# Jax-Rene/monitor-systam-flink-quickstart

Hardware: AMD Instinct MI355X
Metric: events/sec (node) + p50 alert latency, 1M-key tumbling window at 1/2/4/8 MI355X (higher is better)
Workload: dtype int64; 1 GPU; global_batch=16777216, seq_len=60000, parallelism=keyBy-a2a1, exchange=none, keyed_state=dense, record_bytes=8, keys=1000000, key_distribution=uniform, device=cuda:0

## Files before the change

csrc/kernels_hip.hip:

```cpp
#include <hip/hip_runtime.h>

#include <cstdlib>

#include <algorithm>
#include <numeric>
#include <stdexcept>
#include <string>

#include "mxs_hip_util.h"
#include "mxs_kernels.h"

namespace mxs {
namespace {

constexpr int kWave = 64;

__device__ __forceinline__ int lane_id() { return threadIdx.x & (kWave - 1); }

__device__ __forceinline__ int64_t wave_max_i64(int64_t v) {
#pragma unroll
  for (int o = 32; o > 0; o >>= 1) {
    int64_t w = __shfl_xor(v, o);
    v = v > w ? v : w;
  }
// ... 770 lines not shown
    if (simple) {
      bool ok = true;
#pragma unroll
      for (int u = 0; u < CU; ++u) {
        const int64_t d = ct[u] - plan.tbase;
        ok = ok && ck[u] < kTombKey && !(plan.drop_late && ct[u] < plan.late_ts) && d >= 0 &&
             d < ((int64_t)1 << 31);
      }
      simple = __all(ok);
    }
    if (RB == 8 && simple) {
#pragma unroll
      for (int u = 0; u < CU; ++u) {
        const uint64_t k = ck[u];
        const int64_t t = ct[u];
        const uint64_t v = cv[u];
        tmax = t > tmax ? t : tmax;
        const uint32_t du = (uint32_t)(t - plan.tbase);
        uint32_t q = (uint32_t)((double)du * plan.inv_pane);
        const uint32_t qp = q * pane_u;
        q = qp > du ? q - 1u : (du - qp >= pane_u ? q + 1u : q);
        qmin32 = q < qmin32 ? q : qmin32;
        pmask |= pane_bit(q);
        qmax32 = q > qmax32 ? q : qmax32;
        flags |= (int64_t)(int32_t)v != (int64_t)v ? 4 : 0;
        uint32_t b;
        if constexpr (ONE) {
          b = sub_of(k, plan);
        } else {
          const int32_t jh = plan.nranks == 1 ? 0
                             : plan.hash_mode ? jhash_tab[k] : java_long_hash((int64_t)k);
          b = kg_lds ? bucket_of(k, jh, plan, skg) : bucket_of(k, jh, plan, kg_dest);
        }
        keep[u] = true;
        bk[u] = b;
        if constexpr (RB == 8) {
          flags |= narrow_fits(k, (int64_t)v, q) ? 0 : 16;
          rec[u] = make_uint2((uint32_t)k, ((uint32_t)v << 4) | (q & 15u));
        } else {
          rec[u] = make_uint4((uint32_t)k, (uint32_t)(k >> 32), (uint32_t)v, q);
        }
        rk[u] = atomicAdd(&rcnt[b], 1u);
      }
    } else
#pragma unroll
    for (int u = 0; u < CU; ++u) {
      const int64_t i = ev_at(r0, u);
      keep[u] = false;
      if (i < end) {
        const uint64_t k = ck[u];
        const int64_t t = ct[u];
        const uint64_t v = cv[u];
        tmax = t > tmax ? t : tmax;
        const PartEval e = ONE      ? part_eval<true>(k, t, jhash_tab, plan, kg_dest)
                           : kg_lds ? part_eval(k, t, jhash_tab, plan, skg)
                                    : part_eval(k, t, jhash_tab, plan, kg_dest);
        if (e.kind == 1) {
          ++nlate;
          if (late_idx) {
            const unsigned long long pos = atomicAdd((unsigned long long*)&stats[kStatLate], 1ull);
            if (pos < late_cap) late_idx[pos] = (uint32_t)i;
          }
        } else if (e.kind >= 2) {
          flags |= e.kind == 2 ? 2 : 8;
        } else {
          if ((int64_t)(int32_t)v != (int64_t)v) flags |= 4;
          qmin32 = e.t < qmin32 ? e.t : qmin32;
          pmask |= pane_bit(e.t);
          qmax32 = e.t > qmax32 ? e.t : qmax32;
          keep[u] = true;
          bk[u] = e.bucket;
          if constexpr (RB == 8) {
            if (!narrow_fits(k, (int64_t)v, e.t)) flags |= 16;
            rec[u] = make_uint2((uint32_t)k, ((uint32_t)v << 4) | (e.t & 15u));
          } else {
            rec[u] = make_uint4((uint32_t)k, (uint32_t)(k >> 32), (uint32_t)v, e.t);
          }
          rk[u] = atomicAdd(&rcnt[e.bucket], 1u);
        }
      }
    }
    __syncthreads();
    const uint32_t myc = threadIdx.x < (unsigned)nb ? rcnt[threadIdx.x] : 0u;
    const uint32_t off = block_exclusive_scan(myc, wsum);
    if (threadIdx.x < (unsigned)nb) {
      roff[threadIdx.x] = off;
      dbase[threadIdx.x] = threadIdx.x * bcap + run_base[threadIdx.x] + lcnt[threadIdx.x] - off;
    }
    __syncthreads();
#pragma unroll
    for (int u = 0; u < CU; ++u)
      if (keep[u]) {
        const uint32_t j = roff[bk[u]] + rk[u];
        rbuf[j] = rec[u];
        sbk[j] = (uint16_t)bk[u];
      }
    __syncthreads();
    const uint32_t nrec = wsum[16];
    nacc += threadIdx.x == 0 ? nrec : 0u;
    if (!any_ovf) {
      RT* outr = (RT*)out;
      for (uint32_t j = threadIdx.x; j < nrec; j += blockDim.x) outr[dbase[sbk[j]] + j] = rbuf[j];
    }
    __syncthreads();
    if (threadIdx.x < (unsigned)nb) {
      lcnt[threadIdx.x] += rcnt[threadIdx.x];
      rcnt[threadIdx.x] = 0;
    }
    __syncthreads();
  }
  if (threadIdx.x < (unsigned)nb && !any_ovf) {
    const int b = threadIdx.x;
    RT* dst = (RT*)out + (size_t)b * bcap + run_base[b];
    RT hole;
    if constexpr (RB == 8) hole = make_uint2(0xFFFFFFFFu, 0xFFFFFFFFu);
    else hole = make_uint4(0xFFFFFFFFu, 0xFFFFFFFFu, 0u, kHoleT);
    for (uint32_t w = lcnt[b]; w < resv[b]; ++w) dst[w] = hole;
  }

  int64_t qmin = qmin32 == 0xFFFFFFFFu && qmax32 == 0 ? INT64_MAX : (int64_t)qmin32;
  int64_t qmax = qmin == INT64_MAX ? INT64_MIN : (int64_t)qmax32;
  tmax = block_reduce_i64(tmax, lred, 0);
  qmin = block_reduce_i64(qmin, lred, 1);
  qmax = block_reduce_i64(qmax, lred, 0);
  pmask = (uint32_t)block_reduce_i64(pmask, lred, 3);
  if (!late_idx) nlate = block_reduce_i64(nlate, lred, 2);
  flags = (any_ovf ? 1 : 0) | block_reduce_i64(flags & 2, lred, 0) |
          block_reduce_i64(flags & 4, lred, 0) | block_reduce_i64(flags & 8, lred, 0) |
          (RB == 8 ? block_reduce_i64(flags & 16, lred, 0) : 0);
  if (threadIdx.x == 0) {
    atomicMax((long long*)&stats[kStatMaxTs], (long long)tmax);
    if (nacc) {
      atomicMin((long long*)&stats[kStatMinPane], (long long)qmin);
      atomicMax((long long*)&stats[kStatMaxPane], (long long)qmax);
      atomicAdd((unsigned long long*)&stats[kStatAccepted], (unsigned long long)nacc);
      if (pmask) atomicOr((unsigned long long*)&stats[kStatPaneMask], (unsigned long long)pmask);
    }
    if (!late_idx && nlate) atomicAdd((unsigned long long*)&stats[kStatLate], (unsigned long long)nlate);
    if (flags) atomicOr((unsigned long long*)&stats[kStatOverflow], (unsigned long long)flags);
  }
}

constexpr int kOpSub = 4;
__device__ __forceinline__ uint32_t wave_inclusive_scan_dpp(uint32_t x) {
  x += (uint32_t)__builtin_amdgcn_update_dpp(0, (int)x, 0x111, 0xF, 0xF, false);
  x += (uint32_t)__builtin_amdgcn_update_dpp(0, (int)x, 0x112, 0xF, 0xF, false);
  x += (uint32_t)__builtin_amdgcn_update_dpp(0, (int)x, 0x114, 0xF, 0xF, false);
  x += (uint32_t)__builtin_amdgcn_update_dpp(0, (int)x, 0x118, 0xF, 0xF, false);
  x += (uint32_t)__builtin_amdgcn_update_dpp(0, (int)x, 0x142, 0xA, 0xF, false);
  x += (uint32_t)__builtin_amdgcn_update_dpp(0, (int)x, 0x143, 0xC, 0xF, false);
  return x;
}
constexpr size_t onepass_lds(int ru) {
  return (size_t)1024 * ru * 8 + (size_t)(3 * kCMaxNb + 4) * 4 + 20 * 4 + 16 * 8;
}
static_assert(kCG == kPartGranule, "reservation granule differs from the host's capacity bound");
static_assert(onepass_lds(kOnePassRound / 1024) <= 160 * 1024, "one-pass round exceeds 160 KiB");

template <int V, int RU, bool K32, bool PAIR>
__global__ __launch_bounds__(1024) void partition_onepass_kernel(
    const uint64_t* __restrict__ keys, const int64_t* __restrict__ ts,
    const uint64_t* __restrict__ vals, int64_t n, int64_t chunk, PartPlan plan,
    uint32_t* __restrict__ cursor, uint2* __restrict__ out, int64_t* __restrict__ stats,
    uint32_t* __restrict__ late_idx, uint32_t late_cap) {
  static_assert(RU % kOpSub == 0, "a round is a whole number of sub-steps");
  constexpr int R = 1024 * RU, NS = RU / kOpSub, SUB = 1024 * kOpSub;
  constexpr uint32_t kDropped = 0xFFFFFFFFu;
  extern __shared__ __attribute__((aligned(16))) unsigned char osm[];
  const int nb = 1 << plan.nsub_log2;
  uint2* rbuf = (uint2*)osm;
  uint32_t* rcnt = (uint32_t*)(rbuf + R);
  uint32_t* roff = rcnt + kCMaxNb;
  uint32_t* gbase = roff + kCMaxNb + 4;
  uint32_t* wsum = gbase + kCMaxNb;
  int64_t* lred = (int64_t*)(wsum + 20);

  for (int b = threadIdx.x; b < kCMaxNb; b += blockDim.x) rcnt[b] = 0;
  if (threadIdx.x == 0) {
    wsum[17] = 0;
    wsum[18] = 0;
    wsum[19] = 0;
  }
  __syncthreads();
  const int64_t start = (int64_t)blockIdx.x * chunk;
  const int64_t end = start + chunk < n ? start + chunk : n;
  const uint32_t bcap = plan.bucket_cap;

  auto tid_now = [&]() -> uint32_t {
    uint32_t t = threadIdx.x;
    asm volatile("" : "+v"(t));
    return t;
  };
  auto ev_off = [&](int u) -> uint32_t {
    if constexpr (PAIR) return (uint32_t)(u >> 1) * 2048u + 2u * tid_now() + (uint32_t)(u & 1);
    else return (uint32_t)u * 1024u + tid_now();
  };
  auto sub_len = [&](int64_t base) -> uint32_t {
    const int64_t rem = end - base;
    return rem <= 0 ? 0u : rem >= SUB ? (uint32_t)SUB : (uint32_t)rem;
  };
  uint64_t nk[kOpSub], nv[kOpSub];
  int64_t nt[kOpSub];
  auto load_half = [&](int64_t base, int h) {
    const uint32_t len = sub_len(base);
    const uint64_t* kb = K32 ? reinterpret_cast<const uint64_t*>(
                                   reinterpret_cast<const int32_t*>(keys) + base)
                             : keys + base;
    const int64_t* tb = ts + base;
    const uint64_t* vb = vals + base;
    if constexpr (PAIR) {
      {
        const int u = 2 * h;
        const uint32_t o = ev_off(u);
        if (o + 1 < len) {
          ldkey2<V, K32>(kb, o, nk[u], nk[u + 1]);
          uint64_t t0, t1;
          ld64x2<V>(tb, o, t0, t1);
          nt[u] = (int64_t)t0;
          nt[u + 1] = (int64_t)t1;
          ld64x2<V>(vb, o, nv[u], nv[u + 1]);
        } else if (o < len) {
          nk[u] = ldkey<V, K32>(kb, o);
          nt[u] = ldin<V>(&tb[o]);
          nv[u] = ldin<V>(&vb[o]);
        }
      }
    } else {
#pragma unroll
      for (int u = 2 * h; u < 2 * h + 2; ++u) {
        const uint32_t o = ev_off(u);
        if (o < len) {
          nk[u] = ldkey<V, K32>(kb, o);
          nt[u] = ldin<V>(&tb[o]);
          nv[u] = ldin<V>(&vb[o]);
        }
      }
    }
  };
  static_assert(kOpSub == 4, "a sub-step is two halves of two events");

  int64_t tmax = INT64_MIN;
  uint32_t nlate = 0, qmin32 = 0xFFFFFFFFu, qmax32 = 0, pmask = 0, flags = 0;
  const bool pane32 = plan.window_mode && plan.pane > 0 && plan.pane < ((int64_t)1 << 31);
  const uint32_t pane_u = (uint32_t)plan.pane;
  load_half(start, 0);
  load_half(start, 1);
  for (int64_t r0 = start; r0 < end; r0 += R) {
    uint2 rec[RU];
    uint32_t br[RU];
#pragma unroll
    for (int s = 0; s < NS; ++s) {
      const int64_t s0 = r0 + (int64_t)s * SUB;
      const uint32_t len = sub_len(s0);
      bool simple = len == (uint32_t)SUB && pane32 && !(plan.ablate & 8u);
      if (simple) {
        int64_t tbase_v = plan.tbase;
        asm volatile("" : "+s"(tbase_v));
        bool ok = true;
#pragma unroll
        for (int u = 0; u < kOpSub; ++u) {
          const int64_t d = nt[u] - tbase_v;
          ok = ok && nk[u] < kTombKey && !(plan.drop_late && nt[u] < plan.late_ts) && d >= 0 &&
               d < ((int64_t)1 << 31);
        }
        simple = __all(ok);
      }
      if (simple) {
#pragma unroll
        for (int u = 0; u < kOpSub; ++u) {
          const uint64_t k = nk[u];
          const int64_t t = nt[u];
          const uint64_t v = nv[u];
          tmax = t > tmax ? t : tmax;
          const uint32_t du = (uint32_t)(t - plan.tbase);
          uint32_t q = (uint32_t)((double)du * plan.inv_pane);
          const uint32_t qp = q * pane_u;
          q = qp > du ? q - 1u : (du - qp >= pane_u ? q + 1u : q);
          qmin32 = q < qmin32 ? q : qmin32;
          pmask |= pane_bit(q);
          qmax32 = q > qmax32 ? q : qmax32;
          flags |= (int64_t)(int32_t)v != (int64_t)v ? 4u : 0u;
          flags |= narrow_fits(k, (int64_t)v, q) ? 0u : 16u;
          const uint32_t b = sub_of(k, plan);
          rec[s * kOpSub + u] = make_uint2((uint32_t)k, ((uint32_t)v << 4) | (q & 15u));
          br[s * kOpSub + u] = (b << 16) | atomicAdd(&rcnt[b], 1u);
          if (u & 1) load_half(s0 + SUB, u >> 1);
          __builtin_amdgcn_sched_barrier(0);
        }
      } else {
#pragma unroll 1
        for (int u = 0; u < kOpSub; ++u) {
          uint64_t k = nk[0], v = nv[0];
          int64_t t = nt[0];
#pragma unroll
          for (int j = 1; j < kOpSub; ++j)
            if (u == j) {
              k = nk[j];
              t = nt[j];
              v = nv[j];
            }
          uint32_t rx = 0, ry = 0, rb = kDropped;
          const uint32_t o = ev_off(u);
          if (o < len) {
            tmax = t > tmax ? t : tmax;
            const PartEval e = part_eval<true>(k, t, nullptr, plan, nullptr);
            if (e.kind == 1) {
              ++nlate;
              if (late_idx) {
                const unsigned long long pos =
                    atomicAdd((unsigned long long*)&stats[kStatLate], 1ull);
                if (pos < late_cap) late_idx[pos] = (uint32_t)(s0 + o);
              }
            } else if (e.kind >= 2) {
              flags |= e.kind == 2 ? 2u : 8u;
            } else {
              if ((int64_t)(int32_t)v != (int64_t)v) flags |= 4u;
              qmin32 = e.t < qmin32 ? e.t : qmin32;
              pmask |= pane_bit(e.t);
              qmax32 = e.t > qmax32 ? e.t : qmax32;
              if (!narrow_fits(k, (int64_t)v, e.t)) flags |= 16u;
              rx = (uint32_t)k;
              ry = ((uint32_t)v << 4) | (e.t & 15u);
              rb = (e.bucket << 16) | atomicAdd(&rcnt[e.bucket], 1u);
            }
          }
#pragma unroll
          for (int j = 0; j < kOpSub; ++j)
            if (u == j) {
              rec[s * kOpSub + j] = make_uint2(rx, ry);
              br[s * kOpSub + j] = rb;
            }
        }
        load_half(s0 + SUB, 0);
        load_half(s0 + SUB, 1);
      }
    }
    __syncthreads();
    const uint32_t tid = tid_now();
    if (tid < 64) {
      const uint4 c0 = ((const uint4*)rcnt)[2 * tid];
      const uint4 c1 = ((const uint4*)rcnt)[2 * tid + 1];
      ((uint4*)rcnt)[2 * tid] = make_uint4(0, 0, 0, 0);
      ((uint4*)rcnt)[2 * tid + 1] = make_uint4(0, 0, 0, 0);
      const uint32_t sum = c0.x + c0.y + c0.z + c0.w + c1.x + c1.y + c1.z + c1.w;
      const uint32_t incl = wave_inclusive_scan_dpp(sum);
      uint4 o0, o1;
      o0.x = incl - sum;
      o0.y = o0.x + c0.x;
      o0.z = o0.y + c0.y;
      o0.w = o0.z + c0.z;
      o1.x = o0.w + c0.w;
      o1.y = o1.x + c1.x;
      o1.z = o1.y + c1.y;
      o1.w = o1.z + c1.z;
      ((uint4*)roff)[2 * tid] = o0;
      ((uint4*)roff)[2 * tid + 1] = o1;
      if (tid == 63) {
        roff[kCMaxNb] = incl;
        wsum[17] += incl;
      }
    }
    __syncthreads();
    uint32_t c4 = 0, gb = 0;
    if (tid < (unsigned)nb) {
      c4 = (roff[tid + 1] - roff[tid] + (kCG - 1)) & ~(uint32_t)(kCG - 1);
      if (c4) gb = atomicAdd(&cursor[tid], c4);
    }
#pragma unroll
    for (int u = 0; u < RU; ++u)
      if (br[u] != kDropped) rbuf[roff[br[u] >> 16] + (br[u] & 0xFFFFu)] = rec[u];
    if (tid < (unsigned)nb) {
      if (c4) {
        if ((uint64_t)gb + c4 > bcap) wsum[18] = 1;
        atomicMax(&wsum[19], gb + c4);
      }
      gbase[tid] = tid * bcap + gb;
    }
    __syncthreads();
    if (!wsum[18]) {
      const int lane = lane_id();
      for (int b = tid >> 6; b < nb; b += 16) {
        const uint32_t o = roff[b], cnt = roff[b + 1] - o;
        const uint32_t cr = (cnt + (kCG - 1)) & ~(uint32_t)(kCG - 1);
        uint4* dst = (uint4*)(out + gbase[b]);
        for (uint32_t j = 2 * lane; j < cr; j += 128) {
          const uint2 a = j < cnt ? rbuf[o + j] : make_uint2(0xFFFFFFFFu, 0xFFFFFFFFu);
          const uint2 c = j + 1 < cnt ? rbuf[o + j + 1] : make_uint2(0xFFFFFFFFu, 0xFFFFFFFFu);
          dst[j >> 1] = make_uint4(a.x, a.y, c.x, c.y);
        }
      }
    }
  }
  __syncthreads();
  const bool any_ovf = wsum[18] != 0;
  const uint32_t nacc = wsum[17];

  int64_t qmin = qmin32 == 0xFFFFFFFFu && qmax32 == 0 ? INT64_MAX : (int64_t)qmin32;
  int64_t qmax = qmin == INT64_MAX ? INT64_MIN : (int64_t)qmax32;
  tmax = block_reduce_i64(tmax, lred, 0);
  qmin = block_reduce_i64(qmin, lred, 1);
  qmax = block_reduce_i64(qmax, lred, 0);
  pmask = (uint32_t)block_reduce_i64(pmask, lred, 3);
  const int64_t nlate_g = late_idx ? 0 : block_reduce_i64(nlate, lred, 2);
  const int64_t fl = (any_ovf ? 1 : 0) | block_reduce_i64(flags, lred, 3);
  if (threadIdx.x == 0) {
    if (wsum[19])
      atomicMax((unsigned long long*)&stats[kStatMaxBucket], (unsigned long long)wsum[19]);
    atomicMax((long long*)&stats[kStatMaxTs], (long long)tmax);
    if (nacc) {
      atomicMin((long long*)&stats[kStatMinPane], (long long)qmin);
      atomicMax((long long*)&stats[kStatMaxPane], (long long)qmax);
      atomicAdd((unsigned long long*)&stats[kStatAccepted], (unsigned long long)nacc);
      if (pmask) atomicOr((unsigned long long*)&stats[kStatPaneMask], (unsigned long long)pmask);
    }
    if (nlate_g) atomicAdd((unsigned long long*)&stats[kStatLate], (unsigned long long)nlate_g);
    if (fl) atomicOr((unsigned long long*)&stats[kStatOverflow], (unsigned long long)fl);
  }
}

__global__ __launch_bounds__(256) void step_begin_kernel(uint32_t* __restrict__ cursor, int nb,
                                                         int64_t* __restrict__ stats) {
  for (int i = blockIdx.x * blockDim.x + threadIdx.x; i < nb; i += gridDim.x * blockDim.x)
    cursor[i] = 0;
  if (blockIdx.x == 0 && threadIdx.x < kStatCount) {
    const int j = threadIdx.x;
    stats[j] = j == kStatMaxTs ? INT64_MIN : j == kStatMinPane ? INT64_MAX
             : j == kStatMaxPane ? INT64_MIN : 0;
  }
}

__global__ void step_finish_kernel(const int64_t* __restrict__ stats, int64_t* __restrict__ local_maxts,
                                   int64_t bound, int32_t event_mode, int64_t proc_now,
                                   int64_t* __restrict__ red, const uint32_t* __restrict__ flags,
                                   int32_t idle, int64_t* __restrict__ host_red, int32_t fill_word,
                                   const uint32_t* __restrict__ cursor, int nb,
                                   uint32_t* __restrict__ next_cursor,
                                   int64_t* __restrict__ next_stats) {
  if (next_cursor) {
    for (int i = threadIdx.x; i < nb; i += blockDim.x) next_cursor[i] = 0;
    if (threadIdx.x < kStatCount) {
      const int j = threadIdx.x;
      next_stats[j] = j == kStatMaxTs ? INT64_MIN : j == kStatMinPane ? INT64_MAX
                    : j == kStatMaxPane ? INT64_MIN : 0;
    }
  }
  __shared__ uint32_t fmax[64];
  if (fill_word) {
    uint32_t m = 0;
    for (int i = threadIdx.x; i < nb; i += 64) m = cursor[i] > m ? cursor[i] : m;
    fmax[threadIdx.x] = m;
    __syncthreads();
    for (int s = 32; s > 0; s >>= 1) {
      if ((int)threadIdx.x < s && fmax[threadIdx.x + s] > fmax[threadIdx.x])
        fmax[threadIdx.x] = fmax[threadIdx.x + s];
      __syncthreads();
    }
  }
  const int j = threadIdx.x;
  if (j >= 16) return;
  int64_t lm = local_maxts[0];
  const int64_t bm = stats[kStatMaxTs];
  lm = bm > lm ? bm : lm;
  if (j == 0) local_maxts[0] = lm;
  const int64_t wm = event_mode ? (lm == INT64_MIN ? INT64_MIN : lm - bound) : proc_now;
  const int64_t ovf = stats[kStatOverflow];
  int64_t v;
  switch (j) {
    case 0: {
      const int64_t qmax = stats[kStatMaxPane];
      v = qmax == INT64_MIN ? INT64_MAX : -qmax;
      break;
    }
    case 1: v = stats[kStatMinPane]; break;
    case 2: v = idle ? INT64_MAX : wm; break;
    case 3:
      v = !fill_word ? -(ovf & 1) : (ovf & 1) ? -((int64_t)1 << 40) : -(int64_t)fmax[0];
      break;
    case 4: v = -((ovf >> 1) & 1); break;
    case 5: v = (ovf & 4) ? -2 : (ovf & 16) ? -1 : 0; break;
    case 6: v = flags ? -(int64_t)(flags[0] & 1u) : 0; break;
    case 7: v = -((ovf >> 3) & 1); break;
    default: v = stats[j - 8]; break;
  }
  red[j] = v;
  if (host_red) host_red[j] = v;
}

__global__ __launch_bounds__(256) void combine_check_kernel(const uint32_t* __restrict__ flags,
                                                            const uint32_t* __restrict__ counts,
                                                            int nb, int64_t* __restrict__ chk) {
  __shared__ uint32_t mx[256];
  __shared__ uint64_t sm[256];
  uint32_t m = 0;
  uint64_t sum = 0;
  for (int i = threadIdx.x; i < nb; i += 256) {
    m = counts[i] > m ? counts[i] : m;
    sum += counts[i];
  }
  mx[threadIdx.x] = m;
  sm[threadIdx.x] = sum;
  __syncthreads();
  for (int s = 128; s > 0; s >>= 1) {
    if ((int)threadIdx.x < s) {
      if (mx[threadIdx.x + s] > mx[threadIdx.x]) mx[threadIdx.x] = mx[threadIdx.x + s];
      sm[threadIdx.x] += sm[threadIdx.x + s];
    }
    __syncthreads();
  }
  if (threadIdx.x == 0) {
    chk[0] = -(int64_t)(flags[0] & 2u);
    chk[1] = -(int64_t)mx[0];
    chk[2] = (int64_t)sm[0];
  }
}

__global__ __launch_bounds__(256) void bucket_repack_kernel(const uint64_t* __restrict__ src,
                                                            const uint32_t* __restrict__ counts,
                                                            uint32_t src_cap, uint32_t dst_cap,
                                                            int words, uint64_t* __restrict__ dst,
                                                            unsigned long long* __restrict__ xstat) {
  const int b = blockIdx.x;
  const uint32_t c = counts[b] < dst_cap ? counts[b] : dst_cap;
  const uint64_t* s = src + (size_t)b * src_cap * words;
  uint64_t* d = dst + (size_t)b * dst_cap * words;
  const size_t nw = (size_t)c * words;
  if (!(((uintptr_t)s | (uintptr_t)d) & 15)) {
    const size_t nv = nw / 2;
    const uint4* s4 = (const uint4*)s;
    uint4* d4 = (uint4*)d;
    for (size_t i = threadIdx.x; i < nv; i += blockDim.x) d4[i] = s4[i];
    if ((nw & 1) && threadIdx.x == 0) d[nw - 1] = s[nw - 1];
  } else {
    for (size_t i = threadIdx.x; i < nw; i += blockDim.x) d[i] = s[i];
  }
  if (xstat && threadIdx.x == 0) {
    atomicAdd(&xstat[1], (unsigned long long)nw * 8ull);
    atomicAdd(&xstat[0], (unsigned long long)dst_cap * words * 8ull);
  }
}

__global__ __launch_bounds__(256) void neg_max_u32_kernel(const uint32_t* __restrict__ counts, int nb,
                                                          int64_t* __restrict__ out) {
  __shared__ uint32_t mx[256];
  uint32_t m = 0;
  for (int i = threadIdx.x; i < nb; i += 256) m = counts[i] > m ? counts[i] : m;
  mx[threadIdx.x] = m;
  __syncthreads();
  for (int s = 128; s > 0; s >>= 1) {
// ... 3420 lines not shown
    }
  }
  auto kfn = partition_compact_kernel<1, kCUProd, ONE, RB, K32, PAIR>;
  static bool attr = false;
  if (!attr) {
    MXS_HIP_CHECK(hipFuncSetAttribute((const void*)kfn, hipFuncAttributeMaxDynamicSharedMemorySize,
                                      (int)compact_lds(kCUProd)));
    attr = true;
  }
  const size_t lds = compact_lds(kCUProd) - (ONE ? (size_t)kKgLdsMax * 4 : 0);
  hipLaunchKernelGGL(kfn, dim3(blocks), dim3(1024), lds, (hipStream_t)stream, keys, ts, vals,
                     jhash_tab, n, chunk, plan, kg_dest, cursor, reinterpret_cast<RecC*>(out),
                     stats, late_idx, late_cap);
  MXS_HIP_CHECK(hipGetLastError());
}

static const bool kPairEnv = getenv_int("MXS_PAIR", 1) != 0;
static const bool kFastEnv = getenv_int("MXS_PART_FAST", 1) != 0;


constexpr int kSplitThreads = 1024;

template <int RB>
struct SplitRec;
template <>
struct SplitRec<8> {
  uint2 r;
  __device__ __forceinline__ void load(const void* base, size_t i) {
    const unsigned long long w =
        __builtin_nontemporal_load(reinterpret_cast<const unsigned long long*>(base) + i);
    r = make_uint2((uint32_t)w, (uint32_t)(w >> 32));
  }
  __device__ __forceinline__ void hole() { r = make_uint2(0xFFFFFFFFu, 0xFFFFFFFFu); }
  __device__ __forceinline__ bool live() const { return (r.y & 15u) != kNarrowHoleT; }
  __device__ __forceinline__ uint64_t key() const { return (uint64_t)r.x; }
  __device__ __forceinline__ void store(void* base, size_t i) const {
    reinterpret_cast<uint2*>(base)[i] = r;
  }
};
template <>
struct SplitRec<24> {
  uint64_t w0, w1, w2;
  __device__ __forceinline__ void load(const void* base, size_t i) {
    const unsigned long long* q = reinterpret_cast<const unsigned long long*>(base) + 3 * i;
    w0 = __builtin_nontemporal_load(q);
    w1 = __builtin_nontemporal_load(q + 1);
    w2 = __builtin_nontemporal_load(q + 2);
  }
  __device__ __forceinline__ void hole() { w0 = w1 = w2 = ~0ull; }
  __device__ __forceinline__ bool live() const { return (uint32_t)w2 != kHoleT; }
  __device__ __forceinline__ uint64_t key() const { return w0; }
  __device__ __forceinline__ void store(void* base, size_t i) const {
    uint64_t* d = reinterpret_cast<uint64_t*>(base) + 3 * i;
    d[0] = w0;
    d[1] = w1;
    d[2] = w2;
  }
};

template <>
struct SplitRec<16> {
  uint4 r;
  __device__ __forceinline__ void load(const void* base, size_t i) {
    const u32x4_t w = __builtin_nontemporal_load(reinterpret_cast<const u32x4_t*>(base) + i);
    r = make_uint4(w.x, w.y, w.z, w.w);
  }
  __device__ __forceinline__ void hole() { r = make_uint4(0xFFFFFFFFu, 0xFFFFFFFFu, 0u, kHoleT); }
  __device__ __forceinline__ bool live() const { return r.w != kHoleT; }
  __device__ __forceinline__ uint64_t key() const { return (uint64_t)r.x | ((uint64_t)r.y << 32); }
  __device__ __forceinline__ void store(void* base, size_t i) const {
    reinterpret_cast<uint4*>(base)[i] = r;
  }
};

template <int RB>
__global__ __launch_bounds__(kSplitThreads) void partition_split_kernel(
    const void* __restrict__ coarse, const uint32_t* __restrict__ coarse_n, uint32_t ccap,
    PartPlan plan, int L, uint32_t* __restrict__ cursor, void* __restrict__ out,
    int64_t* __restrict__ stats) {
  __shared__ uint32_t scnt[32];
  __shared__ uint32_t sovf;
  const uint32_t c = blockIdx.x;
  const uint32_t nf = 1u << L, fmask = nf - 1u;
  if (threadIdx.x < nf) scnt[threadIdx.x] = 0;
  if (threadIdx.x == 0) sovf = 0;
  __syncthreads();
  uint32_t n = coarse_n[c];
  n = n < ccap ? n : ccap;
  const size_t src0 = (size_t)c * ccap;
  const uint32_t bcap = plan.bucket_cap;
  const unsigned long long lt = (1ull << lane_id()) - 1ull;
  bool ovf = false;
  for (uint32_t base = 0; base < n; base += kSplitThreads * 4) {
    SplitRec<RB> r[4];
#pragma unroll
    for (int u = 0; u < 4; ++u) {
      const uint32_t e = base + u * kSplitThreads + threadIdx.x;
      if (e < n)
        r[u].load(coarse, src0 + e);
      else
        r[u].hole();
    }
#pragma unroll
    for (int u = 0; u < 4; ++u) {
      const bool live = r[u].live();
      const uint32_t f = live ? sub_of(r[u].key(), plan) & fmask : 0xFFFFFFFFu;
      unsigned long long todo = __ballot(live);
      while (todo) {
        const int leader = __ffsll((long long)todo) - 1;
        const uint32_t fl = __shfl(f, leader);
        const unsigned long long m = __ballot(live && f == fl);
        uint32_t b = 0;
        if (lane_id() == leader) b = atomicAdd(&scnt[fl], (uint32_t)__popcll(m));
        b = __shfl(b, leader);
        if (live && f == fl) {
          const uint32_t pos = b + (uint32_t)__popcll(m & lt);
          if (pos < bcap)
            r[u].store(out, (size_t)((c << L) | fl) * bcap + pos);
          else
            ovf = true;
        }
        todo &= ~m;
      }
    }
  }
  if (ovf) sovf = 1;
  __syncthreads();
  if (threadIdx.x < nf) cursor[(c << L) | threadIdx.x] = scnt[threadIdx.x];
  if (threadIdx.x == 0 && sovf)
    atomicOr((unsigned long long*)&stats[kStatOverflow], 1ull);
}

static bool pair_aligned(const uint64_t* keys, const int64_t* ts, const uint64_t* vals, bool key32) {
  return ((uintptr_t)ts % 16 == 0) && ((uintptr_t)vals % 16 == 0) &&
         ((uintptr_t)keys % (key32 ? 8 : 16) == 0) && kPairEnv;
}

static bool onepass_ok(const PartPlan& plan, const void* out) {
  return plan.rec_words == 1 && plan.nranks == 1 && plan.nsub_log2 >= 0 &&
         (1 << plan.nsub_log2) <= kCMaxNb && plan.bucket_cap % kCG == 0 &&
         (uintptr_t)out % 16 == 0 &&
         ((uint64_t)plan.bucket_cap << plan.nsub_log2) < (1ull << 32);
}

template <int RU>
void launch_onepass(const uint64_t* keys, const int64_t* ts, const uint64_t* vals, int64_t n,
                    int64_t chunk, int blocks, const PartPlan& plan, uint32_t* cursor, Rec* out,
                    int64_t* stats, uint32_t* late_idx, uint32_t late_cap, intptr_t stream) {
  PartPlan pl = plan;
  if (!kFastEnv) pl.ablate |= 8u;
  const bool pair = pair_aligned(keys, ts, vals, plan.key32) && (blocks == 1 || chunk % 2 == 0);
#define MXS_ONEPASS(K32_, PAIR_)                                                                \
  do {                                                                                          \
    auto kfn = partition_onepass_kernel<1, RU, K32_, PAIR_>;                                    \
    static bool attr = false;                                                                   \
    if (!attr) {                                                                                \
      MXS_HIP_CHECK(hipFuncSetAttribute((const void*)kfn, hipFuncAttributeMaxDynamicSharedMemorySize, \
                                        (int)onepass_lds(RU)));                                 \
      attr = true;                                                                              \
    }                                                                                           \
    hipLaunchKernelGGL(kfn, dim3(blocks), dim3(1024), onepass_lds(RU), (hipStream_t)stream,      \
                       keys, ts, vals, n, chunk, pl, cursor, reinterpret_cast<uint2*>(out),      \
                       stats, late_idx, late_cap);                                               \
  } while (0)
  if (plan.key32) {
    if (pair) MXS_ONEPASS(true, true);
    else MXS_ONEPASS(true, false);
  } else {
    if (pair) MXS_ONEPASS(false, true);
    else MXS_ONEPASS(false, false);
  }
#undef MXS_ONEPASS
  MXS_HIP_CHECK(hipGetLastError());
}

template <bool ONE, int RB>
void dispatch_compact(const uint64_t* keys, const int64_t* ts, const uint64_t* vals,
                      const int32_t* jhash_tab, int64_t n, const PartPlan& plan,
                      const int32_t* kg_dest, uint32_t* cursor, Rec* out, int64_t* stats,
                      uint32_t* late_idx, uint32_t late_cap, intptr_t stream,
                      bool allow_onepass = true) {
  const PartGrid grid = compact_part_grid(n);
  const int blocks = grid.blocks;
  int64_t chunk = grid.chunk;
  const bool pair = pair_aligned(keys, ts, vals, plan.key32);
  if (pair) chunk = (chunk + 1) & ~(int64_t)1;
  if constexpr (ONE && RB == 8) {
    static const bool onepass = getenv_int("MXS_PART_ONEPASS", 1) != 0;
    if (onepass && allow_onepass && onepass_ok(plan, out)) {
      launch_onepass<kOnePassRound / 1024>(keys, ts, vals, n, chunk, blocks, plan, cursor, out,
                                           stats, late_idx, late_cap, stream);
      return;
    }
  }
  PartPlan pl = plan;
  if (!kFastEnv) pl.ablate |= 8u;
#define MXS_COMPACT(K32_, PAIR_)                                                                \
  launch_compact<ONE, RB, K32_, PAIR_>(keys, ts, vals, jhash_tab, n, chunk, blocks, pl,          \
                                       kg_dest, cursor, out, stats, late_idx, late_cap, stream)
  if (plan.key32) {
    if (pair) MXS_COMPACT(true, true);
    else MXS_COMPACT(true, false);
  } else {
    if (pair) MXS_COMPACT(false, true);
    else MXS_COMPACT(false, false);
  }
#undef MXS_COMPACT
}

void partition(const uint64_t* keys, const int64_t* ts, const uint64_t* vals,
               const int32_t* jhash_tab, int64_t n, const PartPlan& plan, const int32_t* kg_dest,
               uint32_t* cursor, Rec* out, int64_t* stats, uint32_t* late_idx, uint32_t late_cap,
               intptr_t stream) {
  const int nb = plan.nranks << plan.nsub_log2;
  if (plan.rec_words == 1) {
    if ((uint64_t)nb * plan.bucket_cap >= (1ull << 32))
      throw std::invalid_argument("partition: 8-byte record buffer above 2^32 records");
    if (plan.nranks != 1) {
      if (nb > kCMaxNb)
        throw std::invalid_argument("partition: 8-byte records to several ranks need <= 512 buckets");
      if (n <= 0) return;
      dispatch_compact<false, 8>(keys, ts, vals, jhash_tab, n, plan, kg_dest, cursor, out, stats,
                                 late_idx, late_cap, stream);
      return;
    }
    if (n <= 0) return;
    if (nb > kCMaxNb && plan.scratch && plan.scratch_cursor && nb <= kCMaxNb * 32) {
      int L = 0;
      while ((nb >> L) > kCMaxNb) ++L;
      PartPlan pc = plan;
      pc.nsub_log2 = plan.nsub_log2 - L;
      pc.bucket_cap = plan.bucket_cap << L;
      hipStream_t st = (hipStream_t)stream;
      MXS_HIP_CHECK(hipMemsetAsync(plan.scratch_cursor, 0, sizeof(uint32_t) * (nb >> L), st));
      dispatch_compact<true, 8>(keys, ts, vals, jhash_tab, n, pc, kg_dest, plan.scratch_cursor,
                                (Rec*)plan.scratch, stats, late_idx, late_cap, stream);
      hipLaunchKernelGGL(partition_split_kernel<8>, dim3(nb >> L), dim3(kSplitThreads), 0, st,
                         (const void*)plan.scratch, plan.scratch_cursor, pc.bucket_cap, plan, L,
                         cursor, (void*)out, stats);
      MXS_HIP_CHECK(hipGetLastError());
      return;
    }
    if (nb > kCMaxNb) {
      if (plan.key32)
        throw std::invalid_argument("partition: int32 keys need <= 512 buckets");
      partition_variant(keys, ts, vals, jhash_tab, n, plan, kg_dest, cursor, out, stats,
                        late_idx, late_cap, stream, 1);
      return;
    }
    dispatch_compact<true, 8>(keys, ts, vals, jhash_tab, n, plan, kg_dest, cursor, out, stats,
                              late_idx, late_cap, stream);
    return;
  }
  if (plan.rec_words == 2 && nb > kCMaxNb && plan.scratch && plan.scratch_cursor &&
      nb <= kCMaxNb * 32 && (uint64_t)nb * plan.bucket_cap < (1ull << 32)) {
    if (n <= 0) return;
    int L = 0;
    while ((nb >> L) > kCMaxNb) ++L;
    PartPlan pc = plan;
    pc.nsub_log2 = plan.nsub_log2 - L;
    pc.bucket_cap = plan.bucket_cap << L;
    if (pc.nsub_log2 < 0) throw std::invalid_argument("two-level partition: too few sub-tables");
    hipStream_t st = (hipStream_t)stream;
    MXS_HIP_CHECK(hipMemsetAsync(plan.scratch_cursor, 0, sizeof(uint32_t) * (nb >> L), st));
    if (plan.nranks == 1)
      dispatch_compact<true, 16>(keys, ts, vals, jhash_tab, n, pc, kg_dest, plan.scratch_cursor,
                                 (Rec*)plan.scratch, stats, late_idx, late_cap, stream);
    else
      dispatch_compact<false, 16>(keys, ts, vals, jhash_tab, n, pc, kg_dest, plan.scratch_cursor,
                                  (Rec*)plan.scratch, stats, late_idx, late_cap, stream);
    hipLaunchKernelGGL(partition_split_kernel<16>, dim3(nb >> L), dim3(kSplitThreads), 0, st,
                       (const void*)plan.scratch, plan.scratch_cursor, pc.bucket_cap, plan, L,
                       cursor, (void*)out, stats);
    MXS_HIP_CHECK(hipGetLastError());
    return;
  }
  if (plan.rec_words == 2 && nb <= kCMaxNb && (uint64_t)nb * plan.bucket_cap < (1ull << 32)) {
    if (n <= 0) return;
    if (plan.nranks == 1)
      dispatch_compact<true, 16>(keys, ts, vals, jhash_tab, n, plan, kg_dest, cursor, out, stats,
                                 late_idx, late_cap, stream);
    else
      dispatch_compact<false, 16>(keys, ts, vals, jhash_tab, n, plan, kg_dest, cursor, out, stats,
                                  late_idx, late_cap, stream);
    return;
  }
  if (plan.key32)
    throw std::invalid_argument("partition: int32 keys need compact records (<= 512 buckets)");
  if (plan.rec_words == 3 && nb > kStageMaxNb && plan.scratch && plan.scratch_cursor &&
      nb <= kStageMaxNb * 32 && (uint64_t)nb * plan.bucket_cap < (1ull << 32)) {
    if (n <= 0) return;
    int L = 0;
    while ((nb >> L) > kStageMaxNb) ++L;
    PartPlan pc = plan;
    pc.nsub_log2 = plan.nsub_log2 - L;
    pc.bucket_cap = plan.bucket_cap << L;
    if (pc.nsub_log2 < 0) throw std::invalid_argument("two-level partition: too few sub-tables");
    hipStream_t st = (hipStream_t)stream;
    MXS_HIP_CHECK(hipMemsetAsync(plan.scratch_cursor, 0, sizeof(uint32_t) * (nb >> L), st));
    partition_variant(keys, ts, vals, jhash_tab, n, pc, kg_dest, plan.scratch_cursor,
                      (Rec*)plan.scratch, stats, late_idx, late_cap, stream, 5);
    hipLaunchKernelGGL(partition_split_kernel<24>, dim3(nb >> L), dim3(kSplitThreads), 0, st,
                       (const void*)plan.scratch, plan.scratch_cursor, pc.bucket_cap, plan, L,
                       cursor, (void*)out, stats);
    MXS_HIP_CHECK(hipGetLastError());
    return;
  }
  partition_variant(keys, ts, vals, jhash_tab, n, plan, kg_dest, cursor, out, stats, late_idx,
                    late_cap, stream, nb <= kStageMaxNb ? 5 : 1);
}

void partition_variant(const uint64_t* keys, const int64_t* ts, const uint64_t* vals,
                       const int32_t* jhash_tab, int64_t n, const PartPlan& plan,
                       const int32_t* kg_dest, uint32_t* cursor, Rec* out, int64_t* stats,
                       uint32_t* late_idx, uint32_t late_cap, intptr_t stream, int variant,
                       int64_t events_per_group) {
  if (n <= 0) return;
  const int nb = plan.nranks << plan.nsub_log2;
  if (nb > 16384) throw std::runtime_error("partition: too many buckets (max 16384)");
  if (variant >= 20 && variant <= 23) {
    if (!onepass_ok(plan, out)) throw std::runtime_error("narrow one-destination variant: plan");
    if (variant == 20) {
      dispatch_compact<true, 8>(keys, ts, vals, jhash_tab, n, plan, kg_dest, cursor, out, stats,
                                late_idx, late_cap, stream, false);
      return;
// ... 1033 lines not shown
```

Baseline: 68.89 billion events/s.

## Double-buffer onepass partition loads and defer per-event stats to block end

Restructures the one-pass partition kernel so event loads for the next sub-step go into an alternate register set (ping-pong), with the first sub-step of the next round prefetched before the scatter barrier. Per-event tmax/qmin/qmax/overflow tracking in the fast path is replaced by running min/max of the time offset and bitwise overflow accumulators, resolved once at kernel end; the slow path reduces through LDS atomics. Adds a DENSE template specialization that computes the bucket with a single multiply and bitfield extract. The cost is more registers for the doubled buffers and more template instantiations, plus subtler correctness reasoning around flag derivation.

```diff
diff --git a/csrc/kernels_hip.hip b/csrc/kernels_hip.hip
--- a/csrc/kernels_hip.hip
+++ b/csrc/kernels_hip.hip
@@ -946,18 +946,26 @@
   return x;
 }
 constexpr size_t onepass_lds(int ru) {
-  return (size_t)1024 * ru * 8 + (size_t)(3 * kCMaxNb + 4) * 4 + 20 * 4 + 16 * 8;
+  return (size_t)1024 * ru * 8 + (size_t)(3 * kCMaxNb + 4) * 4 + 24 * 4 + 17 * 8;
 }
 static_assert(kCG == kPartGranule, "reservation granule differs from the host's capacity bound");
 static_assert(onepass_lds(kOnePassRound / 1024) <= 160 * 1024, "one-pass round exceeds 160 KiB");
 
-template <int V, int RU, bool K32, bool PAIR>
+template <int V, typename T>
+__device__ __forceinline__ T ldoff(const void* base, uint32_t byte_off) {
+  return ldvec<V>(reinterpret_cast<const T*>(reinterpret_cast<const char*>(base) + byte_off));
+}
+__device__ __forceinline__ uint64_t u64_of(uint32_t lo, uint32_t hi) {
+  return (uint64_t)lo | ((uint64_t)hi << 32);
+}
+
+template <int V, int RU, bool K32, bool PAIR, bool DENSE>
 __global__ __launch_bounds__(1024) void partition_onepass_kernel(
     const uint64_t* __restrict__ keys, const int64_t* __restrict__ ts,
     const uint64_t* __restrict__ vals, int64_t n, int64_t chunk, PartPlan plan,
     uint32_t* __restrict__ cursor, uint2* __restrict__ out, int64_t* __restrict__ stats,
     uint32_t* __restrict__ late_idx, uint32_t late_cap) {
-  static_assert(RU % kOpSub == 0, "a round is a whole number of sub-steps");
+  static_assert(RU % (2 * kOpSub) == 0, "a round is an even number of sub-steps");
   constexpr int R = 1024 * RU, NS = RU / kOpSub, SUB = 1024 * kOpSub;
   constexpr uint32_t kDropped = 0xFFFFFFFFu;
   extern __shared__ __attribute__((aligned(16))) unsigned char osm[];
@@ -967,13 +975,19 @@
   uint32_t* roff = rcnt + kCMaxNb;
   uint32_t* gbase = roff + kCMaxNb + 4;
   uint32_t* wsum = gbase + kCMaxNb;
-  int64_t* lred = (int64_t*)(wsum + 20);
+  int64_t* lred = (int64_t*)(wsum + 24);
+  int64_t* ltmax = lred + 16;
 
   for (int b = threadIdx.x; b < kCMaxNb; b += blockDim.x) rcnt[b] = 0;
   if (threadIdx.x == 0) {
     wsum[17] = 0;
     wsum[18] = 0;
     wsum[19] = 0;
+    wsum[20] = 0;
+    wsum[21] = 0;
+    wsum[22] = 0xFFFFFFFFu;
+    wsum[23] = 0;
+    *ltmax = INT64_MIN;
   }
   __syncthreads();
   const int64_t start = (int64_t)blockIdx.x * chunk;
@@ -993,109 +1007,178 @@
     const int64_t rem = end - base;
     return rem <= 0 ? 0u : rem >= SUB ? (uint32_t)SUB : (uint32_t)rem;
   };
-  uint64_t nk[kOpSub], nv[kOpSub];
-  int64_t nt[kOpSub];
-  auto load_half = [&](int64_t base, int h) {
-    const uint32_t len = sub_len(base);
-    const uint64_t* kb = K32 ? reinterpret_cast<const uint64_t*>(
-                                   reinterpret_cast<const int32_t*>(keys) + base)
-                             : keys + base;
-    const int64_t* tb = ts + base;
-    const uint64_t* vb = vals + base;
+  using KeyReg = std::conditional_t<K32, int32_t, uint64_t>;
+  KeyReg ak[kOpSub], bk[kOpSub];
+  uint64_t av[kOpSub], bv[kOpSub];
+  int64_t at[kOpSub], bt[kOpSub];
+  auto load_none = [&](auto& nk, auto& nt, auto& nv) __attribute__((always_inline)) {
+    auto one = [&](const int u) __attribute__((always_inline)) {
+      asm volatile("" : "=v"(nk[u]));
+      asm volatile("" : "=v"(nt[u]));
+      asm volatile("" : "=v"(nv[u]));
+    };
+    one(0);
+    one(1);
+    one(2);
+    one(3);
+  };
+  auto load_steady = [&](auto& nk, auto& nt, auto& nv, int64_t base) __attribute__((always_inline)) {
+    const char* kb = reinterpret_cast<const char*>(keys) + base * (K32 ? 4 : 8);
+    const char* tb = reinterpret_cast<const char*>(ts + base);
+    const char* vb = reinterpret_cast<const char*>(vals + base);
+    const uint32_t lane = tid_now();
     if constexpr (PAIR) {
-      {
+      auto half = [&](const int h) __attribute__((always_inline)) {
         const int u = 2 * h;
-        const uint32_t o = ev_off(u);
-        if (o + 1 < len) {
-          ldkey2<V, K32>(kb, o, nk[u], nk[u + 1]);
-          uint64_t t0, t1;
-          ld64x2<V>(tb, o, t0, t1);
-          nt[u] = (int64_t)t0;
-          nt[u + 1] = (int64_t)t1;
-          ld64x2<V>(vb, o, nv[u], nv[u + 1]);
-        } else if (o < len) {
-          nk[u] = ldkey<V, K32>(kb, o);
-          nt[u] = ldin<V>(&tb[o]);
-          nv[u] = ldin<V>(&vb[o]);
+        if constexpr (K32) {
+          const u32x2_t w = ldoff<V, u32x2_t>(kb, lane * 8u + h * 2048u * 4u);
+          nk[u] = (int32_t)w.x;
+          nk[u + 1] = (int32_t)w.y;
+        } else {
+          const u32x4_t w = ldoff<V, u32x4_t>(kb, lane * 16u + h * 2048u * 8u);
+          nk[u] = u64_of(w.x, w.y);
+          nk[u + 1] = u64_of(w.z, w.w);
         }
-      }
+        const u32x4_t wt = ldoff<V, u32x4_t>(tb, lane * 16u + h * 2048u * 8u);
+        nt[u] = (int64_t)u64_of(wt.x, wt.y);
+        nt[u + 1] = (int64_t)u64_of(wt.z, wt.w);
+        const u32x4_t wv = ldoff<V, u32x4_t>(vb, lane * 16u + h * 2048u * 8u);
+        nv[u] = u64_of(wv.x, wv.y);
+        nv[u + 1] = u64_of(wv.z, wv.w);
+      };
+      half(0);
+      half(1);
     } else {
-#pragma unroll
-      for (int u = 2 * h; u < 2 * h + 2; ++u) {
-        const uint32_t o = ev_off(u);
-        if (o < len) {
-          nk[u] = ldkey<V, K32>(kb, o);
-          nt[u] = ldin<V>(&tb[o]);
-          nv[u] = ldin<V>(&vb[o]);
-        }
-      }
+      auto one = [&](const int u) __attribute__((always_inline)) {
+        if constexpr (K32) nk[u] = ldoff<V, int32_t>(kb, lane * 4u + u * 1024u * 4u);
+        else nk[u] = ldoff<V, uint64_t>(kb, lane * 8u + u * 1024u * 8u);
+        nt[u] = ldoff<V, int64_t>(tb, lane * 8u + u * 1024u * 8u);
+        nv[u] = ldoff<V, uint64_t>(vb, lane * 8u + u * 1024u * 8u);
+      };
+      one(0);
+      one(1);
+      one(2);
+      one(3);
     }
   };
-  static_assert(kOpSub == 4, "a sub-step is two halves of two events");
-
-  int64_t tmax = INT64_MIN;
-  uint32_t nlate = 0, qmin32 = 0xFFFFFFFFu, qmax32 = 0, pmask = 0, flags = 0;
+  static_assert(kOpSub == 4, "the loads and the general path name four events");
+
+  uint32_t dmin = 0xFFFFFFFFu, dmax = 0, pmask = 0;
+  bool fast_seen = false;
   const bool pane32 = plan.window_mode && plan.pane > 0 && plan.pane < ((int64_t)1 << 31);
   const uint32_t pane_u = (uint32_t)plan.pane;
-  load_half(start, 0);
-  load_half(start, 1);
-  for (int64_t r0 = start; r0 < end; r0 += R) {
-    uint2 rec[RU];
-    uint32_t br[RU];
-#pragma unroll
-    for (int s = 0; s < NS; ++s) {
-      const int64_t s0 = r0 + (int64_t)s * SUB;
-      const uint32_t len = sub_len(s0);
-      bool simple = len == (uint32_t)SUB && pane32 && !(plan.ablate & 8u);
+  auto pane_of = [&](uint32_t du) __attribute__((always_inline)) -> uint32_t {
+    const uint32_t q = (uint32_t)((double)du * plan.inv_pane);
+    const uint32_t qp = q * pane_u;
+    const uint32_t dec = qp > du ? 1u : 0u;
+    const uint32_t inc = (du - qp >= pane_u ? 1u : 0u) & ~dec;
+    return q - dec + inc;
+  };
+  const bool late_on = plan.drop_late != 0;
+  const uint32_t nsub = (uint32_t)plan.nsub_log2;
+  const uint32_t bsh = ((DENSE ? (uint32_t)plan.dense_bits : 32u) - nsub) & 31u;
+  auto bucket_of_key = [&](uint64_t k) __attribute__((always_inline)) -> uint32_t {
+    uint32_t h;
+    if constexpr (DENSE) {
+      h = (uint32_t)k * plan.dense_mul;
+    } else {
+      h = (uint32_t)k * 0x9E3779B1u ^ (uint32_t)(k >> 32) * 0x85EBCA77u;
+      h ^= h >> 15;
+      h *= 0x2C1B3C6Du;
+      h ^= h >> 13;
+    }
+    return __builtin_amdgcn_ubfe(h, bsh, nsub);
+  };
+
+  uint2 rec[RU];
+  uint32_t br[RU];
+  auto substep = [&](auto& ck, auto& ct, auto& cv, auto& xk, auto& xt, auto& xv, const int s,
+                     const int64_t r0) __attribute__((always_inline)) {
+    const int64_t s0 = r0 + (int64_t)s * SUB;
+    const uint32_t len = sub_len(s0);
+    bool simple = false;
+    if (len == (uint32_t)SUB) {
+      if (s != NS - 1) {
+        const int64_t last = PAIR ? (end - SUB) & ~(int64_t)1 : end - SUB;
+        load_steady(xk, xt, xv, s0 + SUB <= last ? s0 + SUB : last);
+        __builtin_amdgcn_sched_barrier(0);
+      }
+      simple = pane32 && !(plan.ablate & 8u);
       if (simple) {
         int64_t tbase_v = plan.tbase;
         asm volatile("" : "+s"(tbase_v));
         bool ok = true;
 #pragma unroll
         for (int u = 0; u < kOpSub; ++u) {
-          const int64_t d = nt[u] - tbase_v;
-          ok = ok && nk[u] < kTombKey && !(plan.drop_late && nt[u] < plan.late_ts) && d >= 0 &&
-               d < ((int64_t)1 << 31);
+          const bool in_range = (uint64_t)(ct[u] - tbase_v) < ((uint64_t)1 << 31);
+          const bool late = late_on & (ct[u] < plan.late_ts);
+          ok = ok & ((uint64_t)(int64_t)ck[u] < kTombKey) & !late & in_range;
         }
         simple = __all(ok);
       }
       if (simple) {
+        fast_seen = true;
+        uint32_t w4 = 0, w16 = 0, kmax = 0;
 #pragma unroll
         for (int u = 0; u < kOpSub; ++u) {
-          const uint64_t k = nk[u];
-          const int64_t t = nt[u];
-          const uint64_t v = nv[u];
-          tmax = t > tmax ? t : tmax;
-          const uint32_t du = (uint32_t)(t - plan.tbase);
-          uint32_t q = (uint32_t)((double)du * plan.inv_pane);
-          const uint32_t qp = q * pane_u;
-          q = qp > du ? q - 1u : (du - qp >= pane_u ? q + 1u : q);
-          qmin32 = q < qmin32 ? q : qmin32;
+          const uint64_t k = (uint64_t)(int64_t)ck[u];
+          const uint32_t vlo = (uint32_t)cv[u], vhi = (uint32_t)(cv[u] >> 32);
+          const uint32_t du = (uint32_t)ct[u] - (uint32_t)plan.tbase;
+          dmin = du < dmin ? du : dmin;
+          dmax = du > dmax ? du : dmax;
+          const uint32_t q = pane_of(du);
           pmask |= pane_bit(q);
-          qmax32 = q > qmax32 ? q : qmax32;
-          flags |= (int64_t)(int32_t)v != (int64_t)v ? 4u : 0u;
-          flags |= narrow_fits(k, (int64_t)v, q) ? 0u : 16u;
-          const uint32_t b = sub_of(k, plan);
-          rec[s * kOpSub + u] = make_uint2((uint32_t)k, ((uint32_t)v << 4) | (q & 15u));
+          const uint32_t vsign = (uint32_t)((int32_t)vlo >> 31);
+          w4 |= vhi ^ vsign;
+          w16 |= (uint32_t)(k >> 32) | ((uint32_t)((int32_t)vlo >> 27) ^ vsign);
+          if constexpr (!K32) kmax = (uint32_t)k > kmax ? (uint32_t)k : kmax;
+          const uint32_t b = bucket_of_key(k);
+          rec[s * kOpSub + u] = make_uint2((uint32_t)k, (vlo << 4) | (q & 15u));
           br[s * kOpSub + u] = (b << 16) | atomicAdd(&rcnt[b], 1u);
-          if (u & 1) load_half(s0 + SUB, u >> 1);
           __builtin_amdgcn_sched_barrier(0);
         }
-      } else {
+        if ((w4 | w16) != 0 || kmax == 0xFFFFFFFFu) atomicOr(&wsum[20], (w4 ? 4u : 0u) | 16u);
+      }
+    } else if (s != NS - 1) {
+      load_none(xk, xt, xv);
+    }
+    {
+      if (!simple) {
+        uint64_t k0, k1, k2, k3, v0, v1, v2, v3;
+        int64_t t0, t1, t2, t3;
+        auto load_event = [&](const int u, uint64_t& k, int64_t& t, uint64_t& v)
+                              __attribute__((always_inline)) {
+          int64_t i = s0 + ev_off(u);
+          i = i < end ? i : end - 1;
+          k = ldkey<V, K32>(keys, i);
+          t = ldin<V>(&ts[i]);
+          v = ldin<V>(&vals[i]);
+        };
+        constexpr bool kLoadAhead = RU >= 16;
+        if constexpr (kLoadAhead) {
+          load_event(0, k0, t0, v0);
+          load_event(1, k1, t1, v1);
+          load_event(2, k2, t2, v2);
+          load_event(3, k3, t3, v3);
+        }
+        uint32_t x0 = 0, x1 = 0, x2 = 0, x3 = 0, y0 = 0, y1 = 0, y2 = 0, y3 = 0;
+        uint32_t b0 = kDropped, b1 = kDropped, b2 = kDropped, b3 = kDropped;
+        int64_t tmax = INT64_MIN;
+        uint32_t nlate = 0, flags = 0, qmin32 = 0xFFFFFFFFu, qmax32 = 0;
 #pragma unroll 1
         for (int u = 0; u < kOpSub; ++u) {
-          uint64_t k = nk[0], v = nv[0];
-          int64_t t = nt[0];
-#pragma unroll
-          for (int j = 1; j < kOpSub; ++j)
-            if (u == j) {
-              k = nk[j];
-              t = nt[j];
-              v = nv[j];
-            }
           uint32_t rx = 0, ry = 0, rb = kDropped;
           const uint32_t o = ev_off(u);
           if (o < len) {
+            uint64_t k, v;
+            int64_t t;
+            if constexpr (kLoadAhead) {
+              k = u == 1 ? k1 : u == 2 ? k2 : u == 3 ? k3 : k0;
+              t = u == 1 ? t1 : u == 2 ? t2 : u == 3 ? t3 : t0;
+              v = u == 1 ? v1 : u == 2 ? v2 : u == 3 ? v3 : v0;
+            } else {
+              load_event(u, k, t, v);
+            }
             tmax = t > tmax ? t : tmax;
             const PartEval e = part_eval<true>(k, t, nullptr, plan, nullptr);
             if (e.kind == 1) {
@@ -1118,16 +1201,31 @@
               rb = (e.bucket << 16) | atomicAdd(&rcnt[e.bucket], 1u);
             }
           }
-#pragma unroll
-          for (int j = 0; j < kOpSub; ++j)
-            if (u == j) {
-              rec[s * kOpSub + j] = make_uint2(rx, ry);
-              br[s * kOpSub + j] = rb;
-            }
+          x0 = u == 0 ? rx : x0, y0 = u == 0 ? ry : y0, b0 = u == 0 ? rb : b0;
+          x1 = u == 1 ? rx : x1, y1 = u == 1 ? ry : y1, b1 = u == 1 ? rb : b1;
+          x2 = u == 2 ? rx : x2, y2 = u == 2 ? ry : y2, b2 = u == 2 ? rb : b2;
+          x3 = u == 3 ? rx : x3, y3 = u == 3 ? ry : y3, b3 = u == 3 ? rb : b3;
         }
-        load_half(s0 + SUB, 0);
-        load_half(s0 + SUB, 1);
-      }
+        rec[s * kOpSub + 0] = make_uint2(x0, y0), br[s * kOpSub + 0] = b0;
+        rec[s * kOpSub + 1] = make_uint2(x1, y1), br[s * kOpSub + 1] = b1;
+        rec[s * kOpSub + 2] = make_uint2(x2, y2), br[s * kOpSub + 2] = b2;
+        rec[s * kOpSub + 3] = make_uint2(x3, y3), br[s * kOpSub + 3] = b3;
+        if (tmax > __atomic_load_n(ltmax, __ATOMIC_RELAXED)) atomicMax((long long*)ltmax, (long long)tmax);
+        if (nlate) atomicAdd(&wsum[21], nlate);
+        if (flags) atomicOr(&wsum[20], flags);
+        if (qmin32 < __atomic_load_n(&wsum[22], __ATOMIC_RELAXED)) atomicMin(&wsum[22], qmin32);
+        if (qmax32 > __atomic_load_n(&wsum[23], __ATOMIC_RELAXED)) atomicMax(&wsum[23], qmax32);
+      }
+    }
+  };
+
+  if (start + SUB <= end) load_steady(ak, at, av, start);
+  else load_none(ak, at, av);
+  for (int64_t r0 = start; r0 < end; r0 += R) {
+#pragma unroll
+    for (int s = 0; s < NS; s += 2) {
+      substep(ak, at, av, bk, bt, bv, s, r0);
+      substep(bk, bt, bv, ak, at, av, s + 1, r0);
     }
     __syncthreads();
     const uint32_t tid = tid_now();
@@ -1163,6 +1261,7 @@
 #pragma unroll
     for (int u = 0; u < RU; ++u)
       if (br[u] != kDropped) rbuf[roff[br[u] >> 16] + (br[u] & 0xFFFFu)] = rec[u];
+    asm volatile("" ::"v"(gb));
     if (tid < (unsigned)nb) {
       if (c4) {
         if ((uint64_t)gb + c4 > bcap) wsum[18] = 1;
@@ -1170,6 +1269,10 @@
       }
       gbase[tid] = tid * bcap + gb;
     }
+    __builtin_amdgcn_sched_barrier(0);
+    if (r0 + R + SUB <= end) load_steady(ak, at, av, r0 + R);
+    else load_none(ak, at, av);
+    __builtin_amdgcn_sched_barrier(0);
     __syncthreads();
     if (!wsum[18]) {
       const int lane = lane_id();
@@ -1188,6 +1291,22 @@
   __syncthreads();
   const bool any_ovf = wsum[18] != 0;
   const uint32_t nacc = wsum[17];
+
+  int64_t tmax = INT64_MIN;
+  uint32_t nlate = 0, qmin32 = 0xFFFFFFFFu, qmax32 = 0, flags = 0;
+  if (fast_seen) {
+    tmax = plan.tbase + (int64_t)dmax;
+    qmin32 = pane_of(dmin);
+    qmax32 = pane_of(dmax);
+    flags = qmax32 >= kNarrowHoleT ? 16u : 0u;
+  }
+  if (threadIdx.x == 0) {
+    tmax = *ltmax > tmax ? *ltmax : tmax;
+    nlate = wsum[21];
+    flags |= wsum[20];
+    qmin32 = wsum[22] < qmin32 ? wsum[22] : qmin32;
+    qmax32 = wsum[23] > qmax32 ? wsum[23] : qmax32;
+  }
 
   int64_t qmin = qmin32 == 0xFFFFFFFFu && qmax32 == 0 ? INT64_MAX : (int64_t)qmin32;
   int64_t qmax = qmin == INT64_MAX ? INT64_MIN : (int64_t)qmax32;
@@ -4914,7 +5033,12 @@
   const bool pair = pair_aligned(keys, ts, vals, plan.key32) && (blocks == 1 || chunk % 2 == 0);
 #define MXS_ONEPASS(K32_, PAIR_)                                                                \
   do {                                                                                          \
-    auto kfn = partition_onepass_kernel<1, RU, K32_, PAIR_>;                                    \
+    if (plan.dense_bits > 0) MXS_ONEPASS_D(K32_, PAIR_, true);                                  \
+    else MXS_ONEPASS_D(K32_, PAIR_, false);                                                     \
+  } while (0)
+#define MXS_ONEPASS_D(K32_, PAIR_, DENSE_)                                                      \
+  do {                                                                                          \
+    auto kfn = partition_onepass_kernel<1, RU, K32_, PAIR_, DENSE_>;                            \
     static bool attr = false;                                                                   \
     if (!attr) {                                                                                \
       MXS_HIP_CHECK(hipFuncSetAttribute((const void*)kfn, hipFuncAttributeMaxDynamicSharedMemorySize, \
@@ -4933,6 +5057,7 @@
     else MXS_ONEPASS(false, false);
   }
 #undef MXS_ONEPASS
+#undef MXS_ONEPASS_D
   MXS_HIP_CHECK(hipGetLastError());
 }
 
```

Result: slower. 65.29 billion events/s (-5.2%).
